# braingeneers/statdepth

Hardware: NVIDIA B200
Metric: BD/MBD depth-evals/sec (higher is better)
Workload: dtype f64

## Files before the change

profiles/slab_probe.py:

```python
import os, sys, json
sys.path.insert(0, '.')
import torch
from statdepth_b200 import _engine as E

n, T = 100_000, int(os.environ.get("PROBE_T", "1024"))
steps = int(os.environ.get("PROBE_STEPS", "10"))
eng = E.get_engine(0)
eng.set_option(E.OPT_PROFILE, 1)
dev = torch.device("cuda", 0)
stream = torch.cuda.ExternalStream(eng.stream(), device=dev)
flush = torch.empty(256 << 20, dtype=torch.uint8, device=dev)
g = torch.Generator(device=dev); g.manual_seed(1)
X = torch.empty((T, n), dtype=torch.float64, device=dev)
for r0 in range(0, T, 128):
    X[r0:r0 + 128] = torch.randn((min(128, T - r0), n), dtype=torch.float64, device=dev, generator=g)
X = X.cumsum(0)
if os.environ.get("PROBE_TIES"):
    X = X.round()
out = torch.zeros(n, dtype=torch.int64, device=dev)
configs = sys.argv[1:] or ["parts:SD_MBD_PATH=parts", "slab:"]
ref = None
KEYS = ("SD_MBD_PATH", "SD_MBD_SLAB_G", "SD_MBD_SLAB_THREADS", "SD_MBD_SLAB_MIN", "SD_MBD_SLAB_HIST_THREADS")
for cfg in configs:
    name, _, envs = cfg.partition(":")
    for k in KEYS:
        os.environ.pop(k, None)
    for kv in filter(None, envs.split(",")):
        k, v = kv.split("=")
        os.environ[k] = v
    for _ in range(3):
        eng.band_depth_counts_dev(X.data_ptr(), T, n, n, out.data_ptr(), None, n, 2, True)
    torch.cuda.synchronize()
    ms, phases, launches = 0.0, {}, 0
    for _ in range(steps):
        flush.fill_(1)
        torch.cuda.synchronize()
        e0, e1 = torch.cuda.Event(enable_timing=True), torch.cuda.Event(enable_timing=True)
        e0.record(stream)
        eng.band_depth_counts_dev(X.data_ptr(), T, n, n, out.data_ptr(), None, n, 2, True)
        e1.record(stream)
        e1.synchronize()
        ms += e0.elapsed_time(e1)
        tm = eng.timings()
        launches = tm["launches"]
        for k, v in eng.phase_ns().items():
            phases[k] = phases.get(k, 0) + v
    res = out.clone()
    same = None if ref is None else bool((res == ref).all().item())
    if ref is None:
        ref = res
    print(json.dumps({"config": name, "env": envs, "ms_per_step": ms / steps, "Mdepth_evals_per_s": n / (ms / steps) / 1e3,
                      "phases_ms": {k: v / steps / 1e6 for k, v in phases.items() if v}, "launches": launches,
                      "fallback_rows": tm["fallback_rows"], "equals_first_config": same,
                      "checksum": int(res.sum().item())}), flush=True)
```

statdepth_b200/csrc/common.cuh:

```cuda
#pragma once
#include <cuda_runtime.h>
#include <stdint.h>
#include <stdio.h>
#include <string.h>
#include <functional>

#include "../../include/statdepth_b200.h"

namespace sd {

typedef long long i64;
typedef unsigned long long u64;
typedef unsigned int u32;

void set_error(const char *fmt, ...);

#define SD_CUDA(call)                                                                            \
    do {                                                                                         \
        cudaError_t _e = (call);                                                                 \
        if (_e != cudaSuccess) {                                                                 \
            sd::set_error("%s:%d: %s -> %s", __FILE__, __LINE__, #call, cudaGetErrorString(_e)); \
            return SD_ERR_CUDA;                                                                  \
        }                                                                                        \
    } while (0)
// ... 46 lines not shown
    NUM_BUFS
};

enum { ST_NONFINITE = 1, ST_INTERNAL = 2, ST_NO_MEMBER = 4, ST_BAD_INPUT = 8 };

__host__ __device__ static inline i64 ceil_div(i64 a, i64 b) { return (a + b - 1) / b; }

__device__ __forceinline__ i64 oos_comb(const i64 m, const int J) {
    if (J == 2) return m * (m - 1) / 2;
    return m < 3 ? 0 : (m * (m - 1) / 2) * (m - 2) / 3;
}

__host__ __device__ static inline u64 sortable_key(double x) {
    if (x == 0.0) x = 0.0;
#ifdef __CUDA_ARCH__
    u64 b = (u64)__double_as_longlong(x);
#else
    u64 b;
    memcpy(&b, &x, 8);
#endif
    const u64 mask = (u64)(-(i64)(b >> 63)) | 0x8000000000000000ull;
    return b ^ mask;
}

}

struct sd_ctx {
    int device = 0;
    int sm_count = 0;
    cudaStream_t stream = nullptr;
    cudaStream_t copy_stream = nullptr;
    cudaEvent_t ev_pipe[4] = {nullptr, nullptr, nullptr, nullptr};
    void *stage[2] = {nullptr, nullptr};
    size_t stage_cap[2] = {0, 0};
    cudaEvent_t ev_stage[2] = {nullptr, nullptr};
    cudaEvent_t ev_slab[2] = {nullptr, nullptr};
    cudaEvent_t ev[4] = {nullptr, nullptr, nullptr, nullptr};
    sd_timings last = {0, 0, 0, 0, 0, 0};
    int bd_impl = SD_BD_AUTO;
    int mbd_force_fallback = 0;
    int mbd_no_wait = 0;
    int profile = 0;
    int simplicial_impl = SD_SIMPLICIAL_AUTO;
    int async_device = 0;
    int pending = 0;
    static const int MAX_PROF = 256;
    cudaEvent_t prof_ev[2 * MAX_PROF] = {};
    int prof_phase[MAX_PROF] = {};
    int prof_n = 0;
    int64_t phase_ns[SD_PHASE_COUNT] = {};
    sd::DevBuf buf[sd::NUM_BUFS];
    int *d_status = nullptr;
    int *h_status = nullptr;
};

namespace sd {

int begin_call(sd_ctx *ctx);
int mark(sd_ctx *ctx, int which);
int end_call(sd_ctx *ctx, bool had_copies);
int check_status(sd_ctx *ctx);
int prof_begin(sd_ctx *ctx, int phase);
int prof_end(sd_ctx *ctx);

int band_depth_device(sd_ctx *ctx, const double *dX, i64 T, i64 n, i64 ld, const i64 *d_q, i64 nq, int j,
                      int relax, i64 *d_out);
bool relaxed_overflows(i64 T, i64 others, int j);
int relaxed_overflow_check(i64 T, i64 others, int j, const char *who);
int mbd_all_device(sd_ctx *ctx, const double *dX, i64 T, i64 n, i64 ld, i64 *d_acc2, i64 *d_acc3,
                   bool accumulate = false, i64 group_rows = 0);
int rank_rows_device(sd_ctx *ctx, const double *dX, i64 T, i64 n, i64 ld, int *d_rank_b, int *d_rank_a);
int rank_block_workspace(sd_ctx *ctx, i64 T, i64 ints_per_row, i64 *RB, int **ws);
using RankBlockFn = std::function<void(i64 r0, i64 rows, const int *rb, const int *ra)>;
int for_each_rank_block(sd_ctx *ctx, const double *dX, i64 T, i64 n, i64 ld, bool want_a, i64 max_rows,
                        const RankBlockFn &consume);
int bd_strict_device(sd_ctx *ctx, const double *dX, i64 T, i64 n, i64 ld, const i64 *d_q, i64 nq, int j,
                     i64 *d_out, u64 *d_hits = nullptr);
int bd_strict_gemm_device(sd_ctx *ctx, const double *dX, i64 T, i64 n, i64 ld, const i64 *d_q, i64 nq,
                          i64 *d_out);
int probe_int8_peak(sd_ctx *ctx, double *ops_per_s);
bool bd_match_supported(i64 T, i64 n);
using StrictFallback = int (*)(sd_ctx *ctx, const double *dX, i64 T, i64 n, i64 ld, const i64 *d_q, i64 nq,
                               i64 *d_out);
int bd_strict_match_device(sd_ctx *ctx, const double *dX, i64 T, i64 n, i64 ld, const i64 *d_q, i64 nq, i64 *d_out,
                           StrictFallback fallback, i64 *n_fallback);
int bd_strict_match_batched_device(sd_ctx *ctx, const double *dXg, i64 nb, i64 T, i64 n, const i64 *d_ql, i64 nqb,
                                   i64 *d_out, StrictFallback fallback);
int transpose_device(sd_ctx *ctx, const double *d_in, i64 rows, i64 cols, i64 ld_in, double *d_out);
int gather_i64_device(sd_ctx *ctx, const i64 *d_src, const i64 *d_idx, i64 nq, i64 *d_out);
int compact_columns_device(sd_ctx *ctx, const double *dX, i64 T, i64 n, const i64 *d_cols, i64 m, double *d_out);
int compact_batches_device(sd_ctx *ctx, const double *dX, i64 T, i64 n, const i64 *d_cols, i64 m, i64 nb,
                           double *d_out);
int l1_device(sd_ctx *ctx, const double *dP, i64 n, int d, const i64 *d_q, i64 nq, double *d_out,
              i64 n_pop = 0);
int oja_device(sd_ctx *ctx, const double *dP, i64 n, int d, const i64 *d_q, i64 nq, const i64 *d_pool,
               i64 npool, double hull_volume, double *d_out);
int cloud_blocks_device(sd_ctx *ctx, const double *dP, int d, const i64 *d_member, const i64 *d_off,
                        const i64 *d_qpos, i64 B, int kind, double tol, const double *d_volume, double *d_out);
int simplicial_device(sd_ctx *ctx, const double *dP, i64 n, int d, const i64 *d_q, i64 nq, double tol,
                      i64 *d_out, bool oos = false);
enum ScReduce { SC_TRIANGLES, SC_HALFSPACE };
int simplicial2_count_device(sd_ctx *ctx, const double *d_pts, i64 n, i64 stride_j, i64 T, const i64 *d_q, i64 nq,
                             double tol, i64 *d_out, i64 m_others = -1, ScReduce reduce = SC_TRIANGLES);
int halfspace1_device(sd_ctx *ctx, const double *dX, i64 T, i64 n, i64 ld, i64 *d_out);
enum ProjKind { PJ_TUKEY, PJ_OUTLYING };
int projection_device(sd_ctx *ctx, const double *dF, i64 N, i64 T, int d, i64 ldX, const double *dU, i64 K,
// ... 29 lines not shown
```

statdepth_b200/csrc/ctx.cu:

```cuda
#include <stdarg.h>

#include <new>

#include "common.cuh"

namespace sd {

static thread_local char g_err[512] = "";

void set_error(const char *fmt, ...) {
    va_list ap;
    va_start(ap, fmt);
    vsnprintf(g_err, sizeof(g_err), fmt, ap);
    va_end(ap);
}

int DevBuf::reserve(size_t bytes) {
    if (bytes <= cap) return SD_OK;
    if (p) {
        cudaFree(p);
        p = nullptr;
        cap = 0;
    }
    size_t want = (bytes + (1u << 20) - 1) & ~((size_t)(1u << 20) - 1);
// ... 163 lines not shown

int compact_columns_device(sd_ctx *ctx, const double *dX, i64 T, i64 n, const i64 *d_cols, i64 m, double *d_out) {
    if (T * m == 0) return SD_OK;
    compact_columns_kernel<<<(unsigned)ceil_div(T * m, 256), 256, 0, ctx->stream>>>(dX, T, n, d_cols, m, d_out);
    ctx->last.launches++;
    SD_CUDA(cudaGetLastError());
    return SD_OK;
}

}

extern "C" {

int sd_abi_version(void) { return SD_ABI_VERSION; }

const char *sd_last_error(void) { return sd::g_err; }

int sd_init(int device, sd_ctx **out) {
    if (!out) {
        sd::set_error("sd_init: out is NULL");
        return SD_ERR_INVALID;
    }
    *out = nullptr;
    int count = 0;
    cudaError_t e = cudaGetDeviceCount(&count);
    if (e != cudaSuccess || count == 0) {
        sd::set_error("sd_init: no CUDA device (%s)", e == cudaSuccess ? "count == 0" : cudaGetErrorString(e));
        return SD_ERR_NO_DEVICE;
    }
    if (device < 0 || device >= count) {
        sd::set_error("sd_init: device %d out of range [0,%d)", device, count);
        return SD_ERR_INVALID;
    }
    cudaDeviceProp prop;
    SD_CUDA(cudaGetDeviceProperties(&prop, device));
    if (prop.major != 10) {
        sd::set_error("sd_init: device %d is sm_%d%d; this library is built for sm_100a (B200) only", device,
                      prop.major, prop.minor);
        return SD_ERR_NO_DEVICE;
    }
    SD_CUDA(cudaSetDevice(device));
    sd_ctx *ctx = new (std::nothrow) sd_ctx();
    if (!ctx) {
        sd::set_error("sd_init: out of host memory");
        return SD_ERR_INVALID;
    }
    ctx->device = device;
    ctx->sm_count = prop.multiProcessorCount;
    SD_CUDA(cudaStreamCreateWithFlags(&ctx->stream, cudaStreamNonBlocking));
    SD_CUDA(cudaStreamCreateWithFlags(&ctx->copy_stream, cudaStreamNonBlocking));
    for (int i = 0; i < 4; ++i) SD_CUDA(cudaEventCreateWithFlags(&ctx->ev_pipe[i], cudaEventDisableTiming));
    for (int i = 0; i < 4; ++i) SD_CUDA(cudaEventCreate(&ctx->ev[i]));
    SD_CUDA(cudaMalloc(&ctx->d_status, 8 * sizeof(int)));
    SD_CUDA(cudaMallocHost(&ctx->h_status, 4 * sizeof(int)));
    memset(ctx->h_status, 0, 4 * sizeof(int));
    *out = ctx;
    return SD_OK;
}

int sd_destroy(sd_ctx *ctx) {
    if (!ctx) return SD_OK;
    cudaSetDevice(ctx->device);
    if (ctx->stream) cudaStreamSynchronize(ctx->stream);
    for (int i = 0; i < sd::NUM_BUFS; ++i) ctx->buf[i].release();
    if (ctx->d_status) cudaFree(ctx->d_status);
    if (ctx->h_status) cudaFreeHost(ctx->h_status);
    for (int i = 0; i < 4; ++i)
        if (ctx->ev[i]) cudaEventDestroy(ctx->ev[i]);
    for (int i = 0; i < 2 * sd_ctx::MAX_PROF; ++i)
        if (ctx->prof_ev[i]) cudaEventDestroy(ctx->prof_ev[i]);
    for (int i = 0; i < 4; ++i)
        if (ctx->ev_pipe[i]) cudaEventDestroy(ctx->ev_pipe[i]);
    for (int i = 0; i < 2; ++i) {
        if (ctx->ev_stage[i]) cudaEventDestroy(ctx->ev_stage[i]);
        if (ctx->stage[i]) cudaFreeHost(ctx->stage[i]);
    }
    for (int i = 0; i < 2; ++i)
        if (ctx->ev_slab[i]) cudaEventDestroy(ctx->ev_slab[i]);
    if (ctx->copy_stream) cudaStreamDestroy(ctx->copy_stream);
    if (ctx->stream) cudaStreamDestroy(ctx->stream);
    delete ctx;
    return SD_OK;
}

int sd_device_info(sd_ctx *ctx, sd_devinfo *out) {
    if (!ctx || !out) {
        sd::set_error("sd_device_info: NULL argument");
        return SD_ERR_INVALID;
    }
    cudaDeviceProp prop;
    SD_CUDA(cudaGetDeviceProperties(&prop, ctx->device));
    out->device = ctx->device;
    out->sm_count = prop.multiProcessorCount;
    out->cc_major = prop.major;
    out->cc_minor = prop.minor;
    out->total_mem = (int64_t)prop.totalGlobalMem;
    strncpy(out->name, prop.name, sizeof(out->name) - 1);
    out->name[sizeof(out->name) - 1] = 0;
    return SD_OK;
}

int sd_set_option(sd_ctx *ctx, int option, int64_t value) {
    if (!ctx) {
        sd::set_error("sd_set_option: NULL context");
        return SD_ERR_INVALID;
    }
    switch (option) {
// ... 74 lines not shown
```

statdepth_b200/csrc/mbd.cu:

```cuda
#include <stdlib.h>

#include "common.cuh"
#include "sortnet.cuh"

namespace sd {

constexpr int CAP = 1024;
constexpr int TARGET_PART = 400;
constexpr int MAX_PARTS = 1024;
constexpr int MAX_SAMPLE = 8192;
constexpr int OVERSAMPLE = 32;
constexpr int KEY_BITS = 22;
constexpr u32 KEY_MAX = (1u << KEY_BITS) - 1u;
constexpr int FB_TILE = 4096;
constexpr int PT_BUCKETS = 1024;

__device__ __forceinline__ i64 comb2_dev(i64 m) { return m * (m - 1) / 2; }
__device__ __forceinline__ i64 comb3_dev(i64 m) {
    return m < 3 ? 0 : (m * (m - 1) / 2) * (m - 2) / 3;
}

constexpr int SP_THREADS = 256;

__device__ __forceinline__ double row_reference(const double *__restrict__ xr, const i64 n) {
// ... 1136 lines not shown
static int pow2ceil_int(i64 v) {
    int p = 1;
    while (p < v) p <<= 1;
    return p;
}

struct SlabPlan {
    bool ok;
    int G, NBc, NB, ecap, threads;
    size_t smem_rank, smem_hist;
};

static int env_int(const char *name, const int fallback) {
    const char *e = getenv(name);
    return e && *e ? atoi(e) : fallback;
}

static SlabPlan slab_plan(const double *dX, const i64 n, const i64 ld) {
    SlabPlan p;
    memset(&p, 0, sizeof(p));
    if (const char *e = getenv("SD_MBD_PATH"))
        if (!strcmp(e, "parts")) return p;
    i64 min_n = env_int("SD_MBD_SLAB_MIN", (int)SL_MIN_N);
    if (min_n < SL_MIN_N) min_n = SL_MIN_N;
    if (n < min_n || n > SL_MAX_N || (ld & 1) || ((uintptr_t)dX & 15)) return p;
    int threads = env_int("SD_MBD_SLAB_THREADS", 1024);
    if (threads < 128 || threads > 1024 || (threads & 31)) threads = 1024;
    const int g_forced = env_int("SD_MBD_SLAB_G", 0);
    const i64 nb0 = ceil_div(n, SL_MEAN);
    const size_t smem_max = 232448 - 256;
    for (int G = 1; G <= 32; ++G) {
        if (g_forced > 0 && G != g_forced) continue;
        i64 NBc = ((ceil_div(nb0, G) + 512) / 1024) * 1024;
        if (NBc < 1024) NBc = 1024;
        if (n > NBc * G * (SL_MEAN + 1) + NBc * G / 2) NBc += 1024;
        const i64 per = ceil_div(n, G);
        const i64 ecap = per + per / 16 + 128;
        if (ecap > 65535 || NBc > 65535) continue;
        const size_t smem = (size_t)(ecap + SL_SORT_CAP) * 4 + (size_t)NBc * 4;
        if (smem > smem_max) continue;
        p.ok = true;
        p.G = G;
        p.NBc = (int)NBc;
        p.NB = (int)(NBc * G);
        p.ecap = (int)ecap;
        p.threads = threads;
        p.smem_rank = smem;
        p.smem_hist = (size_t)p.NB * 4;
        break;
    }
    return p;
}

struct PartPlan {
    int P, S;
    i64 NP, row_stride, Tc;
    bool rank_subbin;
    float *part_x, *splitters_f;
    unsigned short *tables;
    u32 *part_j, *pbase;
    int *cursor, *rowflag;
    int2 *biglist;
};

static int slab_block(sd_ctx *ctx, const SlabPlan &sp, SlabArgs sa, const RankOut &o, const bool extra,
                      const double *Xb, const i64 r0, const i64 rows, const int **only, bool *done) {
    cudaStream_t st = ctx->stream;
    sa.X = Xb;
    sa.row0 = r0;
    SD_CUDA(cudaMemsetAsync(sa.failcount, 0, sizeof(int), st));
    for (int k = 0; k < 2; ++k)
        if (!ctx->ev_slab[k]) SD_CUDA(cudaEventCreateWithFlags(&ctx->ev_slab[k], cudaEventDisableTiming));
    SD_TRY(prof_begin(ctx, SD_PHASE_MBD_SLAB_HIST));
    mbd_slab_table_kernel<<<(unsigned)rows, SL_TABLE_THREADS, 0, st>>>(sa);
    const bool ask = !ctx->mbd_no_wait;
    if (ask) {
        SD_CUDA(cudaMemcpyAsync(ctx->h_status + 3, sa.failcount, sizeof(int), cudaMemcpyDeviceToHost, st));
        SD_CUDA(cudaEventRecord(ctx->ev_slab[0], st));
    }
    if (env_int("SD_MBD_SLAB_HIST_THREADS", rows <= (i64)ctx->sm_count ? 1024 : SL_HIST_THREADS) == 1024)
        mbd_slab_hist_kernel<1024><<<(unsigned)rows, 1024, sp.smem_hist, st>>>(sa);
    else
        mbd_slab_hist_kernel<SL_HIST_THREADS><<<(unsigned)rows, SL_HIST_THREADS, sp.smem_hist, st>>>(sa);
    SD_TRY(prof_end(ctx));
    ctx->last.launches += 2;
    if (ask) {
        SD_CUDA(cudaMemcpyAsync(ctx->h_status + 2, sa.failcount, sizeof(int), cudaMemcpyDeviceToHost, st));
        SD_CUDA(cudaEventRecord(ctx->ev_slab[1], st));
        SD_CUDA(cudaEventSynchronize(ctx->ev_slab[0]));
        if ((i64)ctx->h_status[3] * 16 > rows) return SD_OK;
    }
    const dim3 sgrid((unsigned)sp.G, (unsigned)rows);
    SD_TRY(prof_begin(ctx, SD_PHASE_MBD_SLAB_RANK));
    if (extra) mbd_slab_rank_kernel<true><<<sgrid, sp.threads, sp.smem_rank, st>>>(sa, o);
    else mbd_slab_rank_kernel<false><<<sgrid, sp.threads, sp.smem_rank, st>>>(sa, o);
    SD_TRY(prof_end(ctx));
    ctx->last.launches++;
    *only = sa.rowflag;
    if (ask) {
        SD_CUDA(cudaEventSynchronize(ctx->ev_slab[1]));
        *done = ctx->h_status[2] == 0;
    }
    return SD_OK;
}

template <bool EXTRA>
static int part_block(sd_ctx *ctx, const PartPlan &pp, const RankOut &o, const double *Xb, const i64 ld,
                      const i64 r0, const i64 rows, const int *only) {
    cudaStream_t st = ctx->stream;
    const i64 n = o.n;
    SD_CUDA(cudaMemsetAsync(pp.cursor, 0, (size_t)pp.Tc * (pp.P + 1) * sizeof(int), st));
    if (pp.P > 1) {
        SD_TRY(prof_begin(ctx, SD_PHASE_MBD_SPLITTERS));
        mbd_splitters_kernel<<<(unsigned)rows, SP_THREADS, 0, st>>>(Xb, n, ld, pp.P, pp.S, pp.splitters_f, pp.tables,
                                                                    pp.rowflag, ctx->d_status, only);
        SD_TRY(prof_end(ctx));
        ctx->last.launches++;
    }
    dim3 pgrid((unsigned)ceil_div(n, PT_CHUNK), (unsigned)rows);
    SD_TRY(prof_begin(ctx, SD_PHASE_MBD_PARTITION));
    mbd_partition_kernel<<<pgrid, PT_THREADS, PT_SMEM, st>>>(Xb, n, ld, pp.P, pp.splitters_f, pp.tables, pp.cursor,
                                                             pp.rowflag, pp.part_x, pp.part_j, pp.row_stride,
                                                             ctx->d_status, only);
    SD_TRY(prof_end(ctx));
    ctx->last.launches++;
    SD_TRY(prof_begin(ctx, SD_PHASE_MBD_RANK));
    int hv_threads = 128;
    while (hv_threads < pp.P) hv_threads <<= 1;
    if (n > 16384) hv_threads = HV_THREADS;
    mbd_heavy_kernel<<<(unsigned)rows, hv_threads, 0, st>>>(Xb, n, ld, pp.P, pp.splitters_f, pp.tables, pp.cursor,
                                                            pp.rowflag, pp.pbase, r0, o, only);
    const RankArgs ra = {pp.P,      pp.cursor, pp.pbase,      pp.rowflag, pp.splitters_f, pp.part_x,   pp.part_j,
                         Xb,        ld,        pp.row_stride, r0,         only,           pp.biglist, ctx->d_status + 2};
    SD_CUDA(cudaMemsetAsync(ctx->d_status + 2, 0, 4 * sizeof(int), st));
    const dim3 rgrid((unsigned)ceil_div(pp.P, RANK_WARPS), (unsigned)rows);
    const unsigned bgrid = (unsigned)(ctx->sm_count * 4);
    const unsigned ogrid = (unsigned)(ctx->sm_count * 8);
    const bool subbin = pp.rank_subbin, split_overflow = subbin && rows * (i64)pp.P >= 100000;
    if (subbin) mbd_rank_subbin_kernel<EXTRA><<<rgrid, RANK_WARPS * 32, 0, st>>>(ra, o);
    else mbd_rank_kernel<EXTRA><<<rgrid, RANK_WARPS * 32, 0, st>>>(ra, o);
    if (split_overflow) mbd_rank_overflow_kernel<EXTRA><<<ogrid, RANK_WARPS * 32, 0, st>>>(ra, o);
    mbd_rank_big_kernel<EXTRA><<<bgrid, RANK_WARPS * 32, 0, st>>>(ra, o, subbin ? (split_overflow ? 2 : 1) : 0);
    SD_TRY(prof_end(ctx));
    ctx->last.launches += split_overflow ? 4 : 3;
    return SD_OK;
}

static int generic_block(sd_ctx *ctx, const PartPlan &pp, const RankOut &o, const double *Xb, const i64 ld,
                         const i64 r0, const i64 rows) {
    if (ctx->mbd_force_fallback) {
        fill_int_kernel<<<(unsigned)ceil_div(rows, 256), 256, 0, ctx->stream>>>(pp.rowflag, rows, 2);
        ctx->last.launches++;
    }
    SD_TRY(prof_begin(ctx, SD_PHASE_MBD_GENERIC));
// ... 19 lines not shown
    const i64 group_rows = o.group_rows;
    if (group_rows < 0 || (group_rows > 0 && T % group_rows != 0)) {
        set_error("mbd: %lld rows are not a multiple of the group size %lld", (long long)T, (long long)group_rows);
        return SD_ERR_INVALID;
    }
    const i64 groups = group_rows > 0 ? T / group_rows : 1;
    const i64 acc_len = n * (groups > 0 ? groups : 1);
    cudaStream_t st = ctx->stream;
    if (!accumulate && d_acc2) {
        if (o.acc3) SD_CUDA(cudaMemsetAsync(o.acc3, 0, (size_t)acc_len * sizeof(i64), st));
        if (T == 0) SD_CUDA(cudaMemsetAsync(d_acc2, 0, (size_t)acc_len * sizeof(i64), st));
    }
    if (T == 0) return SD_OK;

    int target = TARGET_PART;
    if (const char *e = getenv("SD_MBD_TARGET_PART")) {
        const int v = atoi(e);
        if (v >= 64 && v <= 512) target = v;
    }
    bool rank_subbin = true;
    if (const char *e = getenv("SD_MBD_RANK")) rank_subbin = strcmp(e, "network") != 0;
    int P = n <= CAP ? 1 : (int)ceil_div(n, target);
    if (P > MAX_PARTS) P = MAX_PARTS;
    int S = 0;
    if (P > 1) {
        S = pow2ceil_int((i64)OVERSAMPLE * P);
        if (S < 1024) S = 1024;
        if (S > MAX_SAMPLE) S = MAX_SAMPLE;
    }
    const i64 NP = pow2ceil_int(n);
    const i64 row_stride = (i64)P * CAP;

    const size_t per_row = (size_t)(row_stride > NP ? row_stride : NP) * 8;
    i64 Tc = (i64)((6ull << 30) / per_row);
    if (Tc < 1) Tc = 1;
    if (Tc > T) Tc = T;
    if (Tc > 65535) Tc = 65535;

    SD_TRY(ctx->buf[BUF_PART_X].reserve((size_t)Tc * (row_stride * 4 > NP * 8 ? row_stride * 4 : NP * 8)));
    SD_TRY(ctx->buf[BUF_PART_J].reserve((size_t)Tc * row_stride * 4));
    SD_TRY(ctx->buf[BUF_CURSOR].reserve((size_t)Tc * (2 * P + 1) * sizeof(int)));
    SD_TRY(ctx->buf[BUF_SPLIT].reserve((size_t)Tc * (P > 1 ? P - 1 : 1) * sizeof(float) +
                                       (size_t)Tc * PT_BUCKETS * sizeof(unsigned short)));
    float *part_x = ctx->buf[BUF_PART_X].as<float>();
    u32 *part_j = ctx->buf[BUF_PART_J].as<u32>();
    int *cursor = ctx->buf[BUF_CURSOR].as<int>();
    int *rowflag = cursor + (size_t)Tc * P;
    u32 *pbase = reinterpret_cast<u32 *>(rowflag + Tc);
    float *splitters_f = ctx->buf[BUF_SPLIT].as<float>();
    unsigned short *tables = reinterpret_cast<unsigned short *>(splitters_f + (size_t)Tc * (P > 1 ? P - 1 : 1));
    SD_TRY(ctx->buf[BUF_WORK].reserve((size_t)Tc * P * sizeof(int2) + (size_t)acc_len * sizeof(u64)));
    int2 *biglist = ctx->buf[BUF_WORK].as<int2>();
    u64 *raw2 = reinterpret_cast<u64 *>(biglist + (size_t)Tc * P);
    if (d_acc2) SD_CUDA(cudaMemsetAsync(raw2, 0, (size_t)acc_len * sizeof(u64), st));

    SD_CUDA(cudaFuncSetAttribute(mbd_partition_kernel, cudaFuncAttributeMaxDynamicSharedMemorySize, (int)PT_SMEM));

    const SlabPlan sp = ctx->mbd_force_fallback ? SlabPlan{} : slab_plan(dX, n, ld);
    SlabArgs sa = {};
    if (sp.ok) {
        const size_t rows_cap = (size_t)Tc;
        const size_t cpitch = (size_t)((n + 3) & ~(i64)3);
        const size_t off_map = rows_cap * cpitch * sizeof(u32);
        const size_t off_tables = off_map + rows_cap * sizeof(double2);
        const size_t off_below = off_tables + rows_cap * SL_BUCKETS * sizeof(uint2);
        const size_t off_flag = off_below + rows_cap * sp.G * sizeof(u32);
        const size_t off_starts = off_flag + rows_cap * sizeof(int);
        SD_TRY(ctx->buf[BUF_SLAB].reserve(off_starts + rows_cap * sp.NB * sizeof(unsigned short)));
        unsigned char *base = ctx->buf[BUF_SLAB].as<unsigned char>();
        sa.n = n;
        sa.ld = ld;
        sa.G = sp.G;
        sa.NBc = sp.NBc;
        sa.ecap = sp.ecap;
        sa.codes = reinterpret_cast<u32 *>(base);
        sa.cpitch = (i64)cpitch;
        sa.rowmap = reinterpret_cast<double2 *>(base + off_map);
        sa.tables = reinterpret_cast<uint2 *>(base + off_tables);
        sa.below = reinterpret_cast<u32 *>(base + off_below);
        sa.rowflag = reinterpret_cast<int *>(base + off_flag);
        sa.starts = reinterpret_cast<unsigned short *>(base + off_starts);
        sa.failcount = ctx->d_status + 6;
        sa.status = ctx->d_status;
        SD_CUDA(cudaFuncSetAttribute(mbd_slab_hist_kernel<SL_HIST_THREADS>, cudaFuncAttributeMaxDynamicSharedMemorySize,
                                     (int)sp.smem_hist));
        SD_CUDA(cudaFuncSetAttribute(mbd_slab_hist_kernel<1024>, cudaFuncAttributeMaxDynamicSharedMemorySize,
                                     (int)sp.smem_hist));
        SD_CUDA(cudaFuncSetAttribute(mbd_slab_rank_kernel<false>, cudaFuncAttributeMaxDynamicSharedMemorySize,
                                     (int)sp.smem_rank));
        SD_CUDA(cudaFuncSetAttribute(mbd_slab_rank_kernel<true>, cudaFuncAttributeMaxDynamicSharedMemorySize,
                                     (int)sp.smem_rank));
    }

    const PartPlan pp = {P, S, NP, row_stride, Tc, rank_subbin, part_x, splitters_f, tables, part_j, pbase, cursor,
                         rowflag, biglist};
    o.raw2 = d_acc2 ? raw2 : nullptr;
    o.n = n;
    o.full2 = (n - 1) * (n - 2) / 2;
    o.full3 = n - 1 < 3 ? 0 : ((n - 1) * (n - 2) / 2) * (n - 3) / 3;
    const bool extra = o.acc3 || o.rank_b || o.group_rows;
    for (i64 r0 = 0; r0 < T; r0 += Tc) {
        const i64 rows = T - r0 < Tc ? T - r0 : Tc;
        const double *Xb = dX + r0 * ld;
        const int *only = nullptr;
        bool done = false;
        if (sp.ok) SD_TRY(slab_block(ctx, sp, sa, o, extra, Xb, r0, rows, &only, &done));
        if (!done && !ctx->mbd_force_fallback)
            SD_TRY(extra ? part_block<true>(ctx, pp, o, Xb, ld, r0, rows, only)
                         : part_block<false>(ctx, pp, o, Xb, ld, r0, rows, only));
        if (!done) SD_TRY(generic_block(ctx, pp, o, Xb, ld, r0, rows));
        SD_CUDA(cudaGetLastError());
    }
    if (d_acc2) {
        mbd_finish_kernel<<<(unsigned)ceil_div(acc_len, 256), 256, 0, st>>>(raw2, d_acc2, acc_len,
                                                                            (group_rows > 0 ? group_rows : T) * o.full2,
                                                                            accumulate ? 1 : 0);
        ctx->last.launches++;
    }
    SD_CUDA(cudaGetLastError());
    return SD_OK;
}

int mbd_all_device(sd_ctx *ctx, const double *dX, i64 T, i64 n, i64 ld, i64 *d_acc2, i64 *d_acc3, bool accumulate,
                   i64 group_rows) {
    RankOut o = {nullptr, d_acc3};
    o.group_rows = group_rows;
    return rank_pipeline(ctx, dX, T, n, ld, d_acc2, accumulate, o);
}

int rank_rows_device(sd_ctx *ctx, const double *dX, i64 T, i64 n, i64 ld, int *d_rank_b, int *d_rank_a) {
    return rank_pipeline(ctx, dX, T, n, ld, nullptr, false, RankOut{nullptr, nullptr, d_rank_b, d_rank_a});
}

constexpr size_t RANK_BLOCK_BUDGET = 1ull << 30;

int rank_block_workspace(sd_ctx *ctx, i64 T, i64 ints_per_row, i64 *RB, int **ws) {
    i64 rb = (i64)(RANK_BLOCK_BUDGET / ((size_t)ints_per_row * sizeof(int)));
    if (rb < 1) rb = 1;
    if (rb > T) rb = T;
    SD_TRY(ctx->buf[BUF_RANKS].reserve((size_t)rb * ints_per_row * sizeof(int)));
    *RB = rb;
    *ws = ctx->buf[BUF_RANKS].as<int>();
    return SD_OK;
}

int for_each_rank_block(sd_ctx *ctx, const double *dX, i64 T, i64 n, i64 ld, bool want_a, i64 max_rows,
                        const RankBlockFn &consume) {
    i64 RB = 0;
    int *rb = nullptr;
    SD_TRY(rank_block_workspace(ctx, T, want_a ? 2 * n : n, &RB, &rb));
    if (RB > max_rows) RB = max_rows;
    int *ra = want_a ? rb + (size_t)RB * n : nullptr;
    for (i64 r0 = 0; r0 < T; r0 += RB) {
        const i64 rows = T - r0 < RB ? T - r0 : RB;
        SD_TRY(rank_rows_device(ctx, dX + r0 * ld, rows, n, ld, rb, ra));
        consume(r0, rows, rb, ra);
        SD_CUDA(cudaGetLastError());
    }
    return SD_OK;
// ... 19 lines not shown
```

statdepth_b200/csrc/mbd_slab.cuh:

```cuda
#pragma once

namespace sd {

constexpr int SL_BUCKETS = 256;
constexpr int SL_SHIFT = 17;
constexpr int SL_IDBITS = 17;
#ifndef SD_SLAB_MEAN
#define SD_SLAB_MEAN 8
#endif
#ifndef SD_SLAB_HIST_MINB
#define SD_SLAB_HIST_MINB 2
#endif
constexpr int SL_MEAN = SD_SLAB_MEAN;
constexpr int SL_SORT_CAP = 16;
constexpr int SL_BIN_MAX = 255;
constexpr int SL_TABLE_THREADS = 256;
constexpr int SL_HIST_THREADS = 512;
constexpr int SL_SAMPLE = 16384;
constexpr int SL_SORTED = 1024;
constexpr int SL_DUPS_MAX = 3;
constexpr int SL_TRIM = 4;
constexpr i64 SL_MIN_N = SL_SAMPLE;
constexpr i64 SL_MAX_N = 1 << SL_IDBITS;
constexpr u32 SL_PAIRWORK_MAX = 1u << 18;
constexpr u32 SL_IDMASK = (1u << SL_IDBITS) - 1u;
constexpr int SL_TOP0 = 0x43300000;

struct SlabArgs {
    const double *X;
    i64 n, ld;
    int G, NBc, ecap;
    double2 *rowmap;
    uint2 *tables;
    u32 *codes;
    i64 cpitch;
    unsigned short *starts;
    u32 *below;
    int *rowflag;
    int *failcount;
    i64 row0;
    int *status;
};

__device__ __forceinline__ int slab_bucket(const double d) {
    return min(max(__double2hiint(d), SL_TOP0), SL_TOP0 + SL_BUCKETS - 1) - SL_TOP0;
}

__device__ __forceinline__ u32 slab_code(const double x, const double s, const double c, const uint2 *tbl) {
    const double d = fma(x, s, c);
    const uint2 e = tbl[slab_bucket(d)];
    return e.x + __umulhi((u32)__double2loint(d), e.y);
}

__device__ __forceinline__ bool slab_nonfinite(const double x) {
    return (__double2hiint(x) & 0x7ff00000) == 0x7ff00000;
}

template <class V, class F>
__device__ __forceinline__ void slab_stream(const V *__restrict__ src, const int count, const int tid, const int nt,
                                            F &&f) {
    const int tiles = count / (4 * nt);
    int p0 = tid;
    if (tiles > 0) {
        V v[4];
#pragma unroll
        for (int u = 0; u < 4; ++u) v[u] = src[p0 + u * nt];
        for (int t = 1; t <= tiles; ++t) {
            V w[4];
            if (t < tiles) {
#pragma unroll
                for (int u = 0; u < 4; ++u) w[u] = src[p0 + (4 + u) * nt];
            }
#pragma unroll
            for (int u = 0; u < 4; ++u) f(v[u], p0 + u * nt);
            p0 += 4 * nt;
            if (t < tiles) {
#pragma unroll
                for (int u = 0; u < 4; ++u) v[u] = w[u];
            }
        }
    }
    for (; p0 < count; p0 += nt) f(src[p0], p0);
}

__device__ __forceinline__ u32 slab_block_scan(const u32 v, u32 *wsum, u32 &total) {
    const int lane = threadIdx.x & 31, wid = threadIdx.x >> 5, nw = blockDim.x >> 5;
    u32 incl = v;
#pragma unroll
    for (int d = 1; d < 32; d <<= 1) {
        const u32 up = __shfl_up_sync(0xffffffffu, incl, d);
        if (lane >= d) incl += up;
    }
    if (lane == 31) wsum[wid] = incl;
    __syncthreads();
    if (wid == 0) {
        const u32 t = lane < nw ? wsum[lane] : 0u;
        u32 sc = t;
#pragma unroll
        for (int d = 1; d < 32; d <<= 1) {
            const u32 up = __shfl_up_sync(0xffffffffu, sc, d);
            if (lane >= d) sc += up;
        }
        wsum[lane] = sc - t;
        if (lane == 31) wsum[32] = sc;
    }
    __syncthreads();
    total = wsum[32];
    const u32 r = incl - v + wsum[wid];
    __syncthreads();
    return r;
}

__global__ void __launch_bounds__(SL_TABLE_THREADS, 4) mbd_slab_table_kernel(const SlabArgs a) {
    __shared__ u32 bh[SL_BUCKETS];
    __shared__ u32 wsum[33];
    __shared__ int s_dups;
    __shared__ float s_q[2];
    const int tid = threadIdx.x;
    const i64 row = blockIdx.x;
    const int n = (int)a.n;
    const double *xr = a.X + row * a.ld;
    const int NB = a.G * a.NBc;
    constexpr int SL_CHUNKS = SL_SAMPLE / SL_TABLE_THREADS;
    const i64 gap = ((i64)n - SL_TABLE_THREADS) / (SL_CHUNKS - 1);

    const double x0 = row_reference(xr, n);
    if (tid < 32) {
        u32 v[32];
        bool bad = false;
#pragma unroll
        for (int i = 0; i < 32; ++i) {
            const int e = tid * 32 + i;
            const double x = xr[(i64)(e >> 4) * gap + ((e & 15) << 4)];
            bad |= slab_nonfinite(x);
            v[i] = f32_sortable(__double2float_rn(x - x0));
        }
        if (bad) atomicOr(a.status, ST_NONFINITE);
        warp_bitonic_sort<32, u32>(v, tid);
        int d = 0;
#pragma unroll
        for (int i = 0; i + 1 < 32; ++i) d += v[i] == v[i + 1];
        d += __shfl_down_sync(0xffffffffu, v[0], 1) == v[31] && tid < 31;
#pragma unroll
        for (int k = 16; k > 0; k >>= 1) d += __shfl_xor_sync(0xffffffffu, d, k);
        const u32 klo = __shfl_sync(0xffffffffu, v[SL_TRIM], 0);
        const u32 khi = __shfl_sync(0xffffffffu, v[31 - SL_TRIM], 31);
        if (tid == 0) {
            s_dups = d;
            s_q[0] = f32_unsortable(klo);
            s_q[1] = f32_unsortable(khi);
        }
    }
    bh[tid] = 0u;
    __syncthreads();
    const double qlo = x0 + (double)s_q[0], qhi = x0 + (double)s_q[1];
    const double span = qhi - qlo;
    const double lo = qlo - 0.35 * span, hi = qhi + 0.35 * span;
    const double s = ((double)(SL_BUCKETS - 2) * 4294967296.0) / (hi - lo);
    const double c = (4503599627370496.0 + 4294967296.0) - lo * s;
    const bool fail = s_dups > SL_DUPS_MAX || !(span > 0.0) || !(s > 0.0) || slab_nonfinite(s) || slab_nonfinite(c);
    if (tid == 0) {
        a.rowflag[row] = fail ? 2 : 0;
        if (fail) atomicAdd(a.failcount, 1);
        else a.rowmap[row] = make_double2(s, c);
    }
    if (fail) return;

    for (int c0 = 0; c0 < SL_CHUNKS; c0 += 16) {
        double v[16];
#pragma unroll
        for (int u = 0; u < 16; ++u) v[u] = xr[(i64)(c0 + u) * gap + tid];
#pragma unroll
        for (int u = 0; u < 16; ++u) atomicAdd(&bh[slab_bucket(fma(v[u], s, c))], 1u);
    }
    __syncthreads();
    const u32 mine = bh[tid];
    u32 total;
    const u32 excl = slab_block_scan(mine, wsum, total);
    const u32 top = ((u32)NB << SL_SHIFT) - 1u;
    const double scl = (double)top / (double)SL_SAMPLE;
    const u32 c0 = min((u32)((double)excl * scl), top);
    const u32 c1 = min((u32)((double)(excl + mine) * scl), top);
    a.tables[row * SL_BUCKETS + tid] = make_uint2(c0, (tid == 0 || tid == SL_BUCKETS - 1) ? 0u : c1 - c0);
}
static_assert(SL_TABLE_THREADS == SL_BUCKETS && SL_SORTED == 1024 && SL_SORTED == 16 * (SL_SAMPLE / SL_TABLE_THREADS) && SL_TRIM < 32,
              "table kernel layout");

template <int NT>
__global__ void __launch_bounds__(NT, NT == SL_HIST_THREADS ? SD_SLAB_HIST_MINB : 1) mbd_slab_hist_kernel(const SlabArgs a) {
    extern __shared__ __align__(16) unsigned char sl_smem[];
    u32 *bins = reinterpret_cast<u32 *>(sl_smem);
    __shared__ uint2 tbl[SL_BUCKETS];
    __shared__ u32 wsum[33];
    __shared__ u32 s_pairwork;
    const int tid = threadIdx.x, nt = NT;
    const i64 row = blockIdx.x;
    if (a.rowflag[row] & 2) return;
    const int n = (int)a.n;
    const double *xr = a.X + row * a.ld;
    const int NB = a.G * a.NBc;
    for (int k = tid; k < SL_BUCKETS; k += nt) tbl[k] = a.tables[row * SL_BUCKETS + k];
    for (int b = tid; b < NB; b += nt) bins[b] = 0u;
    if (tid == 0) s_pairwork = 0u;
    const double2 sc = a.rowmap[row];
    const double s = sc.x, c = sc.y;
    __syncthreads();

    bool bad = false;
    u32 *crow = a.codes + row * a.cpitch;
    uint2 *crow2 = reinterpret_cast<uint2 *>(crow);
    slab_stream(reinterpret_cast<const double2 *>(xr), n >> 1, tid, nt, [&](const double2 v, const int p) {
        bad |= slab_nonfinite(v.x) | slab_nonfinite(v.y);
        const u32 c0 = slab_code(v.x, s, c, tbl), c1 = slab_code(v.y, s, c, tbl);
        crow2[p] = make_uint2(c0, c1);
        atomicAdd(&bins[c0 >> SL_SHIFT], 1u);
        atomicAdd(&bins[c1 >> SL_SHIFT], 1u);
    });
    if ((n & 1) && tid == 0) {
        bad |= slab_nonfinite(xr[n - 1]);
        const u32 c0 = slab_code(xr[n - 1], s, c, tbl);
        crow[n - 1] = c0;
        atomicAdd(&bins[c0 >> SL_SHIFT], 1u);
    }
    if (bad) atomicOr(a.status, ST_NONFINITE);
    __syncthreads();

    const int bpt = (NB + nt - 1) / nt;
    const int b0 = tid * bpt, b1 = min(b0 + bpt, NB);
    u32 sum = 0u, maxc = 0u, pairwork = 0u;
    for (int b = b0; b < b1; ++b) {
        const u32 cnt = bins[b];
        sum += cnt;
        maxc = max(maxc, cnt);
        if (cnt > (u32)SL_SORT_CAP) pairwork += min(cnt, 65535u) * min(cnt, 65535u);
    }
    if (pairwork) atomicAdd(&s_pairwork, min(pairwork, SL_PAIRWORK_MAX + 1u));
    u32 total;
    u32 run = slab_block_scan(sum, wsum, total);
    for (int b = b0; b < b1; ++b) {
        const u32 cnt = bins[b];
        bins[b] = run;
        run += cnt;
    }
    __syncthreads();
    bool fail = maxc > (u32)SL_BIN_MAX || total != (u32)n;
    if (tid < a.G) {
        const u32 first = bins[tid * a.NBc];
        const u32 next = tid + 1 < a.G ? bins[(tid + 1) * a.NBc] : (u32)n;
        fail |= next - first > (u32)a.ecap;
        a.below[row * a.G + tid] = first;
    }
    if (tid == 0) fail |= s_pairwork > SL_PAIRWORK_MAX;
    fail = __syncthreads_or(fail);
    if (fail) {
        if (tid == 0) {
            a.rowflag[row] = 2;
            atomicAdd(a.failcount, 1);
        }
        return;
    }
    if (b0 < b1) {
        int edge = (b0 / a.NBc) * a.NBc;
        u32 first = bins[edge];
        __syncwarp();
        for (int b = b0; b < b1; ++b) {
            if (b == edge + a.NBc) {
                edge = b;
                first = bins[b];
            }
            if (b != edge) bins[b] -= first;
        }
    }
    __syncthreads();
    if (tid < a.G) bins[tid * a.NBc] = 0u;
    __syncthreads();
    u32 *st2 = reinterpret_cast<u32 *>(a.starts + row * NB);
    for (int w = tid; w < (NB >> 1); w += nt) st2[w] = bins[2 * w] | (bins[2 * w + 1] << 16);
}

template <bool EXTRA>
__device__ __noinline__ void slab_rank_entry(const u32 *ents, const int start, const int cnt, const int m,
                                             const double *__restrict__ xr, const u32 before, const RankOut &o,
                                             const i64 row_global, const i64 acc_off) {
    const u32 mine = ents[start + m];
    const u32 km = mine >> SL_IDBITS;
    u32 less = 0u, eq = 1u;
    for (int f = 0; f < cnt; ++f) {
        const u32 other = ents[start + f];
        const u32 ko = other >> SL_IDBITS;
        less += ko < km;
        if (ko == km && f != m) {
            const double xo = xr[other & SL_IDMASK], xm = xr[mine & SL_IDMASK];
            less += xo < xm;
            eq += xo == xm;
        }
    }
    const u32 b = before + less;
    emit_rank<EXTRA>(o, row_global, acc_off, mine & SL_IDMASK, b, (u32)o.n - b - eq);
}

__device__ __forceinline__ void slab_keep(const u32 code, const u32 id, const u32 word_sa, const u32 ents_sa,
                                          const u32 base_bin, const u32 NBc) {
    const u32 own = (code >> SL_SHIFT) - base_bin;
    if (own < NBc) {
        u32 pos;
        asm volatile("atom.shared.add.u32 %0, [%1], 1;" : "=r"(pos) : "r"(word_sa + 4u * own) : "memory");
        asm volatile("st.shared.u32 [%0], %1;" ::"r"(ents_sa + 4u * pos), "r"(((code << 14) & 0x7ffe0000u) | id)
                     : "memory");
    }
}

template <bool EXTRA>
__global__ void __launch_bounds__(1024, 1) mbd_slab_rank_kernel(const SlabArgs a, const RankOut o) {
    extern __shared__ __align__(16) unsigned char sl_smem[];
    u32 *ents = reinterpret_cast<u32 *>(sl_smem);
    u32 *word = ents + a.ecap + SL_SORT_CAP;
    const int tid = threadIdx.x, nt = blockDim.x, lane = tid & 31, wid = tid >> 5, nw = nt >> 5;
    const i64 row = blockIdx.y;
    const int g = blockIdx.x;
    if (a.rowflag[row] & 2) return;
    const int n = (int)a.n;
    const int NBc = a.NBc;
    const double *xr = a.X + row * a.ld;
    {
        const unsigned short *st = a.starts + (row * a.G + g) * NBc;
        for (int b = tid; b < NBc; b += nt) word[b] = st[b];
    }
    const u32 bel = a.below[row * a.G + g];
    const u32 base_bin = (u32)g * (u32)NBc;
    __syncthreads();
// ... 66 lines not shown
```

Baseline: 86.16 million.

## Report slab fail counts via mapped host memory and replicate bucket tables

Removes per-block memset and device-to-host memcpy of the slab fail counter. The last block of each kernel now writes the count into mapped pinned host memory, and accumulator zeroing moves into the table kernel. Function attributes are set once per context rather than every call. The hist kernel keeps 16 copies of the bucket table in shared memory to cut bank conflicts, and rewrites the bin scan as a warp-strided shuffle scan that subtracts group offsets while packing starts. The trade is more shared memory and a last-block atomic protocol that depends on memory fences.

```diff
diff --git a/profiles/slab_probe.py b/profiles/slab_probe.py
--- a/profiles/slab_probe.py
+++ b/profiles/slab_probe.py
@@ -1,4 +1,4 @@
-import os, sys, json
+import os, sys, json, statistics
 sys.path.insert(0, '.')
 import torch
 from statdepth_b200 import _engine as E
@@ -18,6 +18,59 @@
 if os.environ.get("PROBE_TIES"):
     X = X.round()
 out = torch.zeros(n, dtype=torch.int64, device=dev)
+
+
+def trace(path):
+    from torch.profiler import profile, ProfilerActivity
+    eng.set_option(E.OPT_PROFILE, 0)
+    for _ in range(3):
+        eng.band_depth_counts_dev(X.data_ptr(), T, n, n, out.data_ptr(), None, n, 2, True)
+    torch.cuda.synchronize()
+    raw = path + ".chrome.json"
+    with profile(activities=[ProfilerActivity.CPU, ProfilerActivity.CUDA]) as prof:
+        for _ in range(steps):
+            flush.fill_(1)
+            torch.cuda.synchronize()
+            eng.band_depth_counts_dev(X.data_ptr(), T, n, n, out.data_ptr(), None, n, 2, True)
+            torch.cuda.synchronize()
+    prof.export_chrome_trace(raw)
+    with open(raw) as f:
+        evs = json.load(f)["traceEvents"]
+    os.remove(raw)
+    dev_ev = sorted((e for e in evs if e.get("ph") == "X" and e.get("cat") in ("kernel", "gpu_memcpy", "gpu_memset")),
+                    key=lambda e: e["ts"])
+    step_list, cur = [], None
+    for e in dev_ev:
+        if "fill" in e["name"].lower() or "Fill" in e["name"]:
+            cur = []
+            step_list.append(cur)
+            continue
+        if cur is not None:
+            cur.append(e)
+    rows = []
+    for acts in step_list:
+        if not acts:
+            continue
+        row, prev_end = [], None
+        for e in acts:
+            row.append({"name": e["name"][:60], "cat": e["cat"], "us": e["dur"],
+                        "gap_before_us": None if prev_end is None else e["ts"] - prev_end})
+            prev_end = e["ts"] + e["dur"]
+        rows.append({"span_us": prev_end - acts[0]["ts"], "busy_us": sum(e["dur"] for e in acts), "acts": row})
+    med = {"span_us": statistics.median(r["span_us"] for r in rows),
+           "busy_us": statistics.median(r["busy_us"] for r in rows),
+           "acts": [{"name": a["name"], "us": statistics.median(r["acts"][i]["us"] for r in rows),
+                     "gap_before_us": None if i == 0 else statistics.median(r["acts"][i]["gap_before_us"] for r in rows)}
+                    for i, a in enumerate(rows[0]["acts"]) if all(len(r["acts"]) == len(rows[0]["acts"]) for r in rows)]}
+    res = {"T": T, "n": n, "steps": len(rows), "gpu": torch.cuda.get_device_name(0), "median": med, "per_step": rows}
+    with open(path, "w") as f:
+        json.dump(res, f, indent=1)
+    print(json.dumps({"trace": path, "median": med}), flush=True)
+
+
+if os.environ.get("PROBE_TRACE"):
+    trace(os.environ["PROBE_TRACE"])
+    sys.exit(0)
 configs = sys.argv[1:] or ["parts:SD_MBD_PATH=parts", "slab:"]
 ref = None
 KEYS = ("SD_MBD_PATH", "SD_MBD_SLAB_G", "SD_MBD_SLAB_THREADS", "SD_MBD_SLAB_MIN", "SD_MBD_SLAB_HIST_THREADS")
diff --git a/statdepth_b200/csrc/common.cuh b/statdepth_b200/csrc/common.cuh
--- a/statdepth_b200/csrc/common.cuh
+++ b/statdepth_b200/csrc/common.cuh
@@ -122,6 +122,8 @@
     sd::DevBuf buf[sd::NUM_BUFS];
     int *d_status = nullptr;
     int *h_status = nullptr;
+    int *h_status_dev = nullptr;
+    int mbd_attributes_set = 0;
 };
 
 namespace sd {
diff --git a/statdepth_b200/csrc/ctx.cu b/statdepth_b200/csrc/ctx.cu
--- a/statdepth_b200/csrc/ctx.cu
+++ b/statdepth_b200/csrc/ctx.cu
@@ -239,7 +239,9 @@
     for (int i = 0; i < 4; ++i) SD_CUDA(cudaEventCreateWithFlags(&ctx->ev_pipe[i], cudaEventDisableTiming));
     for (int i = 0; i < 4; ++i) SD_CUDA(cudaEventCreate(&ctx->ev[i]));
     SD_CUDA(cudaMalloc(&ctx->d_status, 8 * sizeof(int)));
-    SD_CUDA(cudaMallocHost(&ctx->h_status, 4 * sizeof(int)));
+    SD_CUDA(cudaMemset(ctx->d_status, 0, 8 * sizeof(int)));
+    SD_CUDA(cudaHostAlloc(&ctx->h_status, 4 * sizeof(int), cudaHostAllocMapped));
+    SD_CUDA(cudaHostGetDevicePointer(&ctx->h_status_dev, ctx->h_status, 0));
     memset(ctx->h_status, 0, 4 * sizeof(int));
     *out = ctx;
     return SD_OK;
diff --git a/statdepth_b200/csrc/mbd.cu b/statdepth_b200/csrc/mbd.cu
--- a/statdepth_b200/csrc/mbd.cu
+++ b/statdepth_b200/csrc/mbd.cu
@@ -1212,6 +1212,22 @@
     return p;
 }
 
+static int mbd_kernel_attributes(sd_ctx *ctx) {
+    if (ctx->mbd_attributes_set) return SD_OK;
+    int optin = 0;
+    SD_CUDA(cudaDeviceGetAttribute(&optin, cudaDevAttrMaxSharedMemoryPerBlockOptin, ctx->device));
+    SD_CUDA(cudaFuncSetAttribute(mbd_partition_kernel, cudaFuncAttributeMaxDynamicSharedMemorySize, (int)PT_SMEM));
+    const void *slab[4] = {(const void *)mbd_slab_hist_kernel<SL_HIST_THREADS>, (const void *)mbd_slab_hist_kernel<1024>,
+                           (const void *)mbd_slab_rank_kernel<false>, (const void *)mbd_slab_rank_kernel<true>};
+    for (const void *f : slab) {
+        cudaFuncAttributes fa;
+        SD_CUDA(cudaFuncGetAttributes(&fa, f));
+        SD_CUDA(cudaFuncSetAttribute(f, cudaFuncAttributeMaxDynamicSharedMemorySize, optin - (int)fa.sharedSizeBytes));
+    }
+    ctx->mbd_attributes_set = 1;
+    return SD_OK;
+}
+
 struct PartPlan {
     int P, S;
     i64 NP, row_stride, Tc;
@@ -1223,32 +1239,28 @@
     int2 *biglist;
 };
 
-static int slab_block(sd_ctx *ctx, const SlabPlan &sp, SlabArgs sa, const RankOut &o, const bool extra,
-                      const double *Xb, const i64 r0, const i64 rows, const int **only, bool *done) {
+static int slab_block(sd_ctx *ctx, const SlabPlan &sp, SlabArgs sa, const SlabReport &rep, const RankOut &o,
+                      const bool extra, const double *Xb, const i64 r0, const i64 rows, const int **only, bool *done) {
     cudaStream_t st = ctx->stream;
     sa.X = Xb;
     sa.row0 = r0;
-    SD_CUDA(cudaMemsetAsync(sa.failcount, 0, sizeof(int), st));
     for (int k = 0; k < 2; ++k)
         if (!ctx->ev_slab[k]) SD_CUDA(cudaEventCreateWithFlags(&ctx->ev_slab[k], cudaEventDisableTiming));
     SD_TRY(prof_begin(ctx, SD_PHASE_MBD_SLAB_HIST));
-    mbd_slab_table_kernel<<<(unsigned)rows, SL_TABLE_THREADS, 0, st>>>(sa);
+    mbd_slab_table_kernel<<<(unsigned)rows, SL_TABLE_THREADS, 0, st>>>(sa, rep);
     const bool ask = !ctx->mbd_no_wait;
-    if (ask) {
-        SD_CUDA(cudaMemcpyAsync(ctx->h_status + 3, sa.failcount, sizeof(int), cudaMemcpyDeviceToHost, st));
-        SD_CUDA(cudaEventRecord(ctx->ev_slab[0], st));
-    }
+    if (ask) SD_CUDA(cudaEventRecord(ctx->ev_slab[0], st));
     if (env_int("SD_MBD_SLAB_HIST_THREADS", rows <= (i64)ctx->sm_count ? 1024 : SL_HIST_THREADS) == 1024)
-        mbd_slab_hist_kernel<1024><<<(unsigned)rows, 1024, sp.smem_hist, st>>>(sa);
+        mbd_slab_hist_kernel<1024><<<(unsigned)rows, 1024, sp.smem_hist, st>>>(sa, rep);
     else
-        mbd_slab_hist_kernel<SL_HIST_THREADS><<<(unsigned)rows, SL_HIST_THREADS, sp.smem_hist, st>>>(sa);
+        mbd_slab_hist_kernel<SL_HIST_THREADS><<<(unsigned)rows, SL_HIST_THREADS, sp.smem_hist, st>>>(sa, rep);
     SD_TRY(prof_end(ctx));
     ctx->last.launches += 2;
+    const volatile int *counts = ctx->h_status + 2;
     if (ask) {
-        SD_CUDA(cudaMemcpyAsync(ctx->h_status + 2, sa.failcount, sizeof(int), cudaMemcpyDeviceToHost, st));
         SD_CUDA(cudaEventRecord(ctx->ev_slab[1], st));
         SD_CUDA(cudaEventSynchronize(ctx->ev_slab[0]));
-        if ((i64)ctx->h_status[3] * 16 > rows) return SD_OK;
+        if ((i64)counts[1] * 16 > rows) return SD_OK;
     }
     const dim3 sgrid((unsigned)sp.G, (unsigned)rows);
     SD_TRY(prof_begin(ctx, SD_PHASE_MBD_SLAB_RANK));
@@ -1259,7 +1271,7 @@
     *only = sa.rowflag;
     if (ask) {
         SD_CUDA(cudaEventSynchronize(ctx->ev_slab[1]));
-        *done = ctx->h_status[2] == 0;
+        *done = counts[0] == 0;
     }
     return SD_OK;
 }
@@ -1385,11 +1397,11 @@
     SD_TRY(ctx->buf[BUF_WORK].reserve((size_t)Tc * P * sizeof(int2) + (size_t)acc_len * sizeof(u64)));
     int2 *biglist = ctx->buf[BUF_WORK].as<int2>();
     u64 *raw2 = reinterpret_cast<u64 *>(biglist + (size_t)Tc * P);
-    if (d_acc2) SD_CUDA(cudaMemsetAsync(raw2, 0, (size_t)acc_len * sizeof(u64), st));
-
-    SD_CUDA(cudaFuncSetAttribute(mbd_partition_kernel, cudaFuncAttributeMaxDynamicSharedMemorySize, (int)PT_SMEM));
+    SD_TRY(mbd_kernel_attributes(ctx));
 
     const SlabPlan sp = ctx->mbd_force_fallback ? SlabPlan{} : slab_plan(dX, n, ld);
+    SlabReport rep = {ctx->h_status_dev + 2, sp.ok && d_acc2 ? raw2 : nullptr, sp.ok && d_acc2 ? acc_len : 0};
+    if (d_acc2 && !sp.ok) SD_CUDA(cudaMemsetAsync(raw2, 0, (size_t)acc_len * sizeof(u64), st));
     SlabArgs sa = {};
     if (sp.ok) {
         const size_t rows_cap = (size_t)Tc;
@@ -1415,14 +1427,6 @@
         sa.starts = reinterpret_cast<unsigned short *>(base + off_starts);
         sa.failcount = ctx->d_status + 6;
         sa.status = ctx->d_status;
-        SD_CUDA(cudaFuncSetAttribute(mbd_slab_hist_kernel<SL_HIST_THREADS>, cudaFuncAttributeMaxDynamicSharedMemorySize,
-                                     (int)sp.smem_hist));
-        SD_CUDA(cudaFuncSetAttribute(mbd_slab_hist_kernel<1024>, cudaFuncAttributeMaxDynamicSharedMemorySize,
-                                     (int)sp.smem_hist));
-        SD_CUDA(cudaFuncSetAttribute(mbd_slab_rank_kernel<false>, cudaFuncAttributeMaxDynamicSharedMemorySize,
-                                     (int)sp.smem_rank));
-        SD_CUDA(cudaFuncSetAttribute(mbd_slab_rank_kernel<true>, cudaFuncAttributeMaxDynamicSharedMemorySize,
-                                     (int)sp.smem_rank));
     }
 
     const PartPlan pp = {P, S, NP, row_stride, Tc, rank_subbin, part_x, splitters_f, tables, part_j, pbase, cursor,
@@ -1437,7 +1441,8 @@
         const double *Xb = dX + r0 * ld;
         const int *only = nullptr;
         bool done = false;
-        if (sp.ok) SD_TRY(slab_block(ctx, sp, sa, o, extra, Xb, r0, rows, &only, &done));
+        if (sp.ok) SD_TRY(slab_block(ctx, sp, sa, rep, o, extra, Xb, r0, rows, &only, &done));
+        rep.zero_len = 0;
         if (!done && !ctx->mbd_force_fallback)
             SD_TRY(extra ? part_block<true>(ctx, pp, o, Xb, ld, r0, rows, only)
                          : part_block<false>(ctx, pp, o, Xb, ld, r0, rows, only));
diff --git a/statdepth_b200/csrc/mbd_slab.cuh b/statdepth_b200/csrc/mbd_slab.cuh
--- a/statdepth_b200/csrc/mbd_slab.cuh
+++ b/statdepth_b200/csrc/mbd_slab.cuh
@@ -42,14 +42,33 @@
     int *status;
 };
 
+struct SlabReport {
+    int *host;
+    u64 *zero;
+    i64 zero_len;
+};
+
 __device__ __forceinline__ int slab_bucket(const double d) {
     return min(max(__double2hiint(d), SL_TOP0), SL_TOP0 + SL_BUCKETS - 1) - SL_TOP0;
 }
 
+constexpr int SL_TBL_COPIES = 16;
+
 __device__ __forceinline__ u32 slab_code(const double x, const double s, const double c, const uint2 *tbl) {
     const double d = fma(x, s, c);
-    const uint2 e = tbl[slab_bucket(d)];
+    const uint2 e = tbl[slab_bucket(d) * SL_TBL_COPIES];
     return e.x + __umulhi((u32)__double2loint(d), e.y);
+}
+
+__device__ __forceinline__ void slab_report(const SlabArgs &a, const SlabReport &r, const bool failed, const bool hist) {
+    if (failed) atomicAdd(a.failcount, 1);
+    __threadfence();
+    if (atomicAdd(a.failcount + 1, 1) != (int)gridDim.x - 1) return;
+    __threadfence();
+    const int count = hist ? atomicExch(a.failcount, 0) : atomicAdd(a.failcount, 0);
+    a.failcount[1] = 0;
+    *(volatile int *)(r.host + (hist ? 0 : 1)) = count;
+    __threadfence_system();
 }
 
 __device__ __forceinline__ bool slab_nonfinite(const double x) {
@@ -111,13 +130,14 @@
     return r;
 }
 
-__global__ void __launch_bounds__(SL_TABLE_THREADS, 4) mbd_slab_table_kernel(const SlabArgs a) {
+__global__ void __launch_bounds__(SL_TABLE_THREADS, 4) mbd_slab_table_kernel(const SlabArgs a, const SlabReport r) {
     __shared__ u32 bh[SL_BUCKETS];
     __shared__ u32 wsum[33];
     __shared__ int s_dups;
     __shared__ float s_q[2];
     const int tid = threadIdx.x;
     const i64 row = blockIdx.x;
+    for (i64 i = row * SL_TABLE_THREADS + tid; i < r.zero_len; i += (i64)gridDim.x * SL_TABLE_THREADS) r.zero[i] = 0ull;
     const int n = (int)a.n;
     const double *xr = a.X + row * a.ld;
     const int NB = a.G * a.NBc;
@@ -161,8 +181,8 @@
     const bool fail = s_dups > SL_DUPS_MAX || !(span > 0.0) || !(s > 0.0) || slab_nonfinite(s) || slab_nonfinite(c);
     if (tid == 0) {
         a.rowflag[row] = fail ? 2 : 0;
-        if (fail) atomicAdd(a.failcount, 1);
-        else a.rowmap[row] = make_double2(s, c);
+        if (!fail) a.rowmap[row] = make_double2(s, c);
+        slab_report(a, r, fail, false);
     }
     if (fail) return;
 
@@ -187,23 +207,29 @@
               "table kernel layout");
 
 template <int NT>
-__global__ void __launch_bounds__(NT, NT == SL_HIST_THREADS ? SD_SLAB_HIST_MINB : 1) mbd_slab_hist_kernel(const SlabArgs a) {
+__global__ void __launch_bounds__(NT, NT == SL_HIST_THREADS ? SD_SLAB_HIST_MINB : 1)
+    mbd_slab_hist_kernel(const SlabArgs a, const SlabReport r) {
     extern __shared__ __align__(16) unsigned char sl_smem[];
     u32 *bins = reinterpret_cast<u32 *>(sl_smem);
-    __shared__ uint2 tbl[SL_BUCKETS];
+    __shared__ uint2 tbl[SL_BUCKETS * SL_TBL_COPIES];
     __shared__ u32 wsum[33];
     __shared__ u32 s_pairwork;
-    const int tid = threadIdx.x, nt = NT;
+    __shared__ u32 s_first[32];
+    const int tid = threadIdx.x, nt = NT, lane = tid & 31, wid = tid >> 5;
     const i64 row = blockIdx.x;
-    if (a.rowflag[row] & 2) return;
+    if (a.rowflag[row] & 2) {
+        if (tid == 0) slab_report(a, r, false, true);
+        return;
+    }
     const int n = (int)a.n;
     const double *xr = a.X + row * a.ld;
     const int NB = a.G * a.NBc;
-    for (int k = tid; k < SL_BUCKETS; k += nt) tbl[k] = a.tables[row * SL_BUCKETS + k];
+    for (int k = tid; k < SL_BUCKETS * SL_TBL_COPIES; k += nt) tbl[k] = a.tables[row * SL_BUCKETS + k / SL_TBL_COPIES];
     for (int b = tid; b < NB; b += nt) bins[b] = 0u;
     if (tid == 0) s_pairwork = 0u;
     const double2 sc = a.rowmap[row];
     const double s = sc.x, c = sc.y;
+    const uint2 *tbl_mine = tbl + (lane & (SL_TBL_COPIES - 1));
     __syncthreads();
 
     bool bad = false;
@@ -211,36 +237,42 @@
     uint2 *crow2 = reinterpret_cast<uint2 *>(crow);
     slab_stream(reinterpret_cast<const double2 *>(xr), n >> 1, tid, nt, [&](const double2 v, const int p) {
         bad |= slab_nonfinite(v.x) | slab_nonfinite(v.y);
-        const u32 c0 = slab_code(v.x, s, c, tbl), c1 = slab_code(v.y, s, c, tbl);
+        const u32 c0 = slab_code(v.x, s, c, tbl_mine), c1 = slab_code(v.y, s, c, tbl_mine);
         crow2[p] = make_uint2(c0, c1);
         atomicAdd(&bins[c0 >> SL_SHIFT], 1u);
         atomicAdd(&bins[c1 >> SL_SHIFT], 1u);
     });
     if ((n & 1) && tid == 0) {
         bad |= slab_nonfinite(xr[n - 1]);
-        const u32 c0 = slab_code(xr[n - 1], s, c, tbl);
+        const u32 c0 = slab_code(xr[n - 1], s, c, tbl_mine);
         crow[n - 1] = c0;
         atomicAdd(&bins[c0 >> SL_SHIFT], 1u);
     }
     if (bad) atomicOr(a.status, ST_NONFINITE);
     __syncthreads();
 
-    const int bpt = (NB + nt - 1) / nt;
-    const int b0 = tid * bpt, b1 = min(b0 + bpt, NB);
+    const int S = NB / (NT / 32);
+    u32 *wbins = bins + wid * S + lane;
     u32 sum = 0u, maxc = 0u, pairwork = 0u;
-    for (int b = b0; b < b1; ++b) {
-        const u32 cnt = bins[b];
+    for (int k = 0; k < S; k += 32) {
+        const u32 cnt = wbins[k];
         sum += cnt;
         maxc = max(maxc, cnt);
         if (cnt > (u32)SL_SORT_CAP) pairwork += min(cnt, 65535u) * min(cnt, 65535u);
     }
     if (pairwork) atomicAdd(&s_pairwork, min(pairwork, SL_PAIRWORK_MAX + 1u));
     u32 total;
-    u32 run = slab_block_scan(sum, wsum, total);
-    for (int b = b0; b < b1; ++b) {
-        const u32 cnt = bins[b];
-        bins[b] = run;
-        run += cnt;
+    u32 run = __shfl_sync(0xffffffffu, slab_block_scan(sum, wsum, total), 0);
+    for (int k = 0; k < S; k += 32) {
+        const u32 cnt = wbins[k];
+        u32 incl = cnt;
+#pragma unroll
+        for (int d = 1; d < 32; d <<= 1) {
+            const u32 up = __shfl_up_sync(0xffffffffu, incl, d);
+            if (lane >= d) incl += up;
+        }
+        wbins[k] = run + incl - cnt;
+        run += __shfl_sync(0xffffffffu, incl, 31);
     }
     __syncthreads();
     bool fail = maxc > (u32)SL_BIN_MAX || total != (u32)n;
@@ -249,33 +281,28 @@
         const u32 next = tid + 1 < a.G ? bins[(tid + 1) * a.NBc] : (u32)n;
         fail |= next - first > (u32)a.ecap;
         a.below[row * a.G + tid] = first;
+        s_first[tid] = first;
     }
     if (tid == 0) fail |= s_pairwork > SL_PAIRWORK_MAX;
     fail = __syncthreads_or(fail);
+    if (tid == 0) slab_report(a, r, fail, true);
     if (fail) {
-        if (tid == 0) {
-            a.rowflag[row] = 2;
-            atomicAdd(a.failcount, 1);
-        }
+        if (tid == 0) a.rowflag[row] = 2;
         return;
     }
-    if (b0 < b1) {
-        int edge = (b0 / a.NBc) * a.NBc;
-        u32 first = bins[edge];
-        __syncwarp();
-        for (int b = b0; b < b1; ++b) {
-            if (b == edge + a.NBc) {
-                edge = b;
-                first = bins[b];
-            }
-            if (b != edge) bins[b] -= first;
-        }
-    }
-    __syncthreads();
-    if (tid < a.G) bins[tid * a.NBc] = 0u;
-    __syncthreads();
+    const uint2 *bins2 = reinterpret_cast<const uint2 *>(bins);
     u32 *st2 = reinterpret_cast<u32 *>(a.starts + row * NB);
-    for (int w = tid; w < (NB >> 1); w += nt) st2[w] = bins[2 * w] | (bins[2 * w + 1] << 16);
+    const int words_c = a.NBc >> 1;
+    int g = 0, edge = words_c;
+    for (int w = tid; w < (NB >> 1); w += nt) {
+        while (w >= edge) {
+            ++g;
+            edge += words_c;
+        }
+        const uint2 v = bins2[w];
+        const u32 first = s_first[g];
+        st2[w] = (v.x - first) | ((v.y - first) << 16);
+    }
 }
 
 template <bool EXTRA>
```

After: 89.34 million (median of 6 runs). 3.7% higher.
